# rpng/open_vins

Hardware: NVIDIA H100
Metric: msckf_updates_per_sec (higher is better)
Workload: dtype f64

## Files before the change

open_vins_b200/csrc/chol_tiles.cuh:

```cuda
#pragma once
#include "chol.cuh"
#ifdef CQ_PROBE
#include <cstdio>
#endif

#define CT_XP 12

__device__ __forceinline__ void ct_dmma(double &d0, double &d1, double a, double b) {
  asm volatile("mma.sync.aligned.m8n8k4.row.col.f64.f64.f64.f64 {%0,%1}, {%2}, {%3}, {%0,%1};" : "+d"(d0), "+d"(d1) : "d"(a), "d"(b));
}
__device__ __forceinline__ void ct_dmma2(double &d0, double &d1, double &e0, double &e1, double a0, double a1, double b) {
  asm volatile("mma.sync.aligned.m16n8k4.row.col.f64.f64.f64.f64 {%0,%1,%2,%3}, {%4,%5}, {%6}, {%0,%1,%2,%3};"
               : "+d"(d0), "+d"(d1), "+d"(e0), "+d"(e1)
               : "d"(a0), "d"(a1), "d"(b));
}
__device__ __forceinline__ void ct_dmma2k8(double &d0, double &d1, double &e0, double &e1, double a00, double a01, double a10, double a11, double b0, double b1) {
  asm volatile("mma.sync.aligned.m16n8k8.row.col.f64.f64.f64.f64 {%0,%1,%2,%3}, {%4,%5,%6,%7}, {%8,%9}, {%0,%1,%2,%3};"
               : "+d"(d0), "+d"(d1), "+d"(e0), "+d"(e1)
               : "d"(a00), "d"(a10), "d"(a01), "d"(a11), "d"(b0), "d"(b1));
}
__device__ __forceinline__ int ct_tri(int b) { return (b * (b + 1)) >> 1; }
__device__ __forceinline__ void ct_bar_group(int id, int nthreads) { asm volatile("bar.sync %0, %1;" ::"r"(id), "r"(nthreads) : "memory"); }
__device__ __forceinline__ size_t ct_idx(int i, int j) { return (size_t)(ct_tri(i >> 3) + (j >> 3)) * 64 + (i & 7) * 8 + (j & 7); }

struct CtView {
  double *T, *Xp0, *Xp1, *invd, *Linv0, *Linv1, *dummyT, *dummyX;
  int *flag;
};
__host__ __device__ inline size_t ct_view_doubles(int NRB) {
  return (size_t)((NRB * (NRB + 1)) / 2) * 64 + 2 * (size_t)NRB * 8 * CT_XP + (size_t)NRB * 8 + 128 + 64 + 2 * CT_XP;
}
__device__ __forceinline__ CtView ct_view_carve(double *base, int NRB, int *flag_word) {
  CtView v;
  v.T = base;
  v.Xp0 = v.T + (size_t)((NRB * (NRB + 1)) / 2) * 64;
  v.Xp1 = v.Xp0 + (size_t)NRB * 8 * CT_XP;
  v.invd = v.Xp1 + (size_t)NRB * 8 * CT_XP;
  v.Linv0 = v.invd + (size_t)NRB * 8;
  v.Linv1 = v.Linv0 + 64;
  v.dummyT = v.Linv1 + 64;
  v.dummyX = v.dummyT + 64;
  v.flag = flag_word;
  return v;
}

__device__ __forceinline__ void ct_diag8_frag(double &d0, double &d1, int nbk, double *invd, bool strict, double floor_d, int *flag) {
  const unsigned full = 0xffffffffu;
  const int lane = threadIdx.x & 31, g = lane >> 2, q = lane & 3;
  bool bad = false;
  double myinv = 0.0;
  const double inv_floor = (floor_d > 0.0) ? fast_rsqrt(floor_d) : 0.0;
  double pj = __shfl_sync(full, d0, 0);
#pragma unroll
  for (int j = 0; j < 8; j++) {
    const int jq = j >> 1;
    const double cur = (j & 1) ? d1 : d0;
    const double ag = __shfl_sync(full, cur, 4 * g + jq);
    const double ac0 = __shfl_sync(full, cur, 8 * q + jq);
    const double ac1 = __shfl_sync(full, cur, 8 * q + 4 + jq);
    double an = 0.0, dn = 0.0;
    if (j < 7) {
      an = __shfl_sync(full, cur, 4 * (j + 1) + jq);
      dn = __shfl_sync(full, ((j + 1) & 1) ? d1 : d0, 4 * (j + 1) + ((j + 1) >> 1));
    }
    const double y = fast_rsqrt(pj);
    const bool in = j < nbk;
    double d, iv;
    if (strict) {
      const bool pos = pj > 0.0;
      bad = bad || (in && !pos);
      d = pj;
      iv = (in && pos) ? y : 0.0;
    } else {
      const bool above = pj > floor_d;
      d = above ? pj : floor_d;
      iv = in ? (above ? y : inv_floor) : 0.0;
    }
    if (j < 7) {
      const double ln = an * iv;
      pj = fma(-ln, ln, dn);
    }
    if (lane == j)
      myinv = iv;
    if (q == jq) {
      if (j & 1)
        d1 = (g == j) ? d * iv : d1 * iv;
      else
        d0 = (g == j) ? d * iv : d0 * iv;
    }
    const double lg = ag * iv, lc0 = ac0 * iv, lc1 = ac1 * iv;
    if (2 * q > j)
      d0 = fma(-lg, lc0, d0);
    if (2 * q + 1 > j)
      d1 = fma(-lg, lc1, d1);
  }
  if (lane < 8)
    invd[lane] = myinv;
  if (bad && lane == 0)
    *flag = 1;
}

__device__ __forceinline__ void ct_linv8(const double *Lt, const double *invd, double *Linv) {
  const int lane = threadIdx.x & 31, cc = lane & 7;
  double mc[8];
#pragma unroll
  for (int j = 0; j < 8; j++) {
    double s0 = (j == cc) ? 1.0 : 0.0, s1 = 0.0;
#pragma unroll
    for (int t = 0; t < j; t++) {
      if (t & 1)
        s1 = fma(-Lt[j * 8 + t], mc[t], s1);
      else
        s0 = fma(-Lt[j * 8 + t], mc[t], s0);
    }
    mc[j] = (s0 + s1) * invd[j];
  }
  if (lane < 8) {
#pragma unroll
    for (int i = 0; i < 8; i++)
      Linv[i * 8 + cc] = (i >= cc) ? mc[i] : 0.0;
  }
}

__device__ __forceinline__ void ct_panel_pair(const CtView &sm, int i, int i1, bool two, int k, const double *Linv, double *Xb) {
  const int lane = threadIdx.x & 31, g = lane >> 2, q = lane & 3;
  double *t = sm.T + (size_t)(ct_tri(i) + k) * 64;
  double *t1 = sm.T + (size_t)(ct_tri(i1) + k) * 64;
  const double a0 = t[g * 8 + q], a1 = t[g * 8 + q + 4];
  const double a10 = two ? t1[g * 8 + q] : 0.0, a11 = two ? t1[g * 8 + q + 4] : 0.0;
  const double b0 = Linv[g * 8 + q], b1 = Linv[g * 8 + q + 4];
  double2 d = make_double2(0.0, 0.0), e = make_double2(0.0, 0.0);
  ct_dmma2k8(d.x, d.y, e.x, e.y, a0, a1, a10, a11, b0, b1);
  *reinterpret_cast<double2 *>(t + 2 * lane) = d;
  *reinterpret_cast<double2 *>(Xb + (size_t)(8 * i + g) * CT_XP + 2 * q) = d;
  if (two) {
    *reinterpret_cast<double2 *>(t1 + 2 * lane) = e;
    *reinterpret_cast<double2 *>(Xb + (size_t)(8 * i1 + g) * CT_XP + 2 * q) = e;
  }
}

__device__ __forceinline__ void ct_panel_rows(double *T, double *Xp, const double *invd, int i0, int stride, int nrows, int k, int nbk) {
  if (i0 >= nrows)
    return;
  const double *Lk = T + (size_t)(ct_tri(k) + k) * 64;
  double L[8][8], iv[8];
#pragma unroll
  for (int c = 0; c < 8; c++) {
    iv[c] = (c < nbk) ? invd[8 * k + c] : 0.0;
#pragma unroll
    for (int t2 = 0; t2 < 4; t2++) {
      if (2 * t2 < c) {
        const double2 v = *reinterpret_cast<const double2 *>(Lk + c * 8 + 2 * t2);
        L[c][2 * t2] = v.x;
        L[c][2 * t2 + 1] = v.y;
      }
    }
  }
  for (int i = i0; i < nrows; i += stride) {
    double *src = T + (size_t)(ct_tri(i >> 3) + k) * 64 + (i & 7) * 8;
    double v[8], x[8];
    {
      const double2 v01 = *reinterpret_cast<const double2 *>(src), v23 = *reinterpret_cast<const double2 *>(src + 2);
      const double2 v45 = *reinterpret_cast<const double2 *>(src + 4), v67 = *reinterpret_cast<const double2 *>(src + 6);
      v[0] = v01.x, v[1] = v01.y, v[2] = v23.x, v[3] = v23.y, v[4] = v45.x, v[5] = v45.y, v[6] = v67.x, v[7] = v67.y;
    }
#pragma unroll
    for (int c = 0; c < 8; c++) {
      x[c] = (c < nbk) ? v[c] * iv[c] : 0.0;
#pragma unroll
      for (int t = c + 1; t < 8; t++)
        v[t] = fma(-x[c], L[t][c], v[t]);
    }
// ... 186 lines not shown
```

open_vins_b200/csrc/k_ekf.cu:

```cuda
#include "chol.cuh"
#include "ovb_internal.cuh"

#define EK_T 32

__global__ void __launch_bounds__(256) k_ekf_gemm(int mode, const double *__restrict__ P, int ldP, const double *__restrict__ H, int ldH,
                                                  const double *__restrict__ Min, int ldM, const DevUpdateInfo *__restrict__ info, int X, int Y,
                                                  int K, double *__restrict__ Cout, int ldC, double sigma2, const double *__restrict__ Rdiag) {
  OVB_PDL_ENTER();
  __shared__ double As[EK_T][EK_T + 1];
  __shared__ double Bs[EK_T][EK_T + 1];
  const int x0 = blockIdx.x * EK_T, y0 = blockIdx.y * EK_T;
  if (mode == 1 && y0 > x0 + EK_T - 1)
    return;
  const int tid = threadIdx.x, tx = tid & 31, ty = tid >> 5;
  double acc[4] = {0, 0, 0, 0};
  const int *cs = info->col_state;
  for (int j0 = 0; j0 < K; j0 += EK_T) {
    for (int e = tid; e < EK_T * EK_T; e += 256) {
      int jj = e >> 5, q = e & 31;
      int j = j0 + jj;
      double av = 0.0, bv = 0.0;
      if (j < K) {
        if (mode == 0) {
          int a = x0 + q;
          if (a < X)
            av = P[(size_t)cs[j] * ldP + a];
        } else {
          int i = x0 + q;
          if (i < X)
            av = H[(size_t)i * ldH + j];
        }
        if (mode == 0) {
          int i = y0 + q;
          if (i < Y)
            bv = H[(size_t)i * ldH + j];
        } else {
          int k = y0 + q;
          if (k < Y)
            bv = Min[(size_t)cs[j] * ldM + k];
        }
      }
      As[jj][q] = av;
      Bs[jj][q] = bv;
    }
    __syncthreads();
#pragma unroll 8
    for (int jj = 0; jj < EK_T; jj++) {
      double b = Bs[jj][tx];
#pragma unroll
      for (int u = 0; u < 4; u++)
        acc[u] += As[jj][ty + 8 * u] * b;
    }
    __syncthreads();
  }
#pragma unroll
  for (int u = 0; u < 4; u++) {
    int x = x0 + ty + 8 * u, y = y0 + tx;
    if (x < X && y < Y) {
      double v = acc[u];
      if (mode == 1 && x == y)
        v += Rdiag ? Rdiag[x] : sigma2;
      Cout[(size_t)x * ldC + y] = v;
    }
  }
}

__global__ void __launch_bounds__(EKC_THREADS) k_ekf_chol(double *__restrict__ S, int ldS, int r, const double *__restrict__ res, double *__restrict__ w,
                                                   double *__restrict__ invdiag, DevUpdateInfo *__restrict__ info, int use_smem) {
  OVB_PDL_ENTER();
  extern __shared__ __align__(16) double chol_sm[];
  __shared__ int flag;
  __shared__ double invd_sh[16];
  const int tid = threadIdx.x;
  if (tid == 0)
    flag = 0;
  for (int j = tid; j < r; j += EKC_THREADS)
    S[(size_t)r * ldS + j] = res[j];
  __syncthreads();
  double *W = S;
  int ld = ldS;
  const int lane = tid & 31, wid = tid >> 5;
  if (use_smem) {
    ld = r | 1;
    W = chol_sm;
    stage_lower_async<EKC_THREADS>(W, ld, S, (size_t)ldS, r + 1, r);
  }
  chol_lower_block<EKC_THREADS, 4>(W, ld, r, 1, &flag, invd_sh, nullptr, 0.0, invdiag);
  __syncthreads();
  if (use_smem) {
    for (int i = wid; i < r; i += EKC_THREADS / 32) {
      for (int j = lane; j <= i; j += 32)
        S[(size_t)i * ldS + j] = W[i * ld + j];
    }
  }
  for (int j = tid; j < r; j += EKC_THREADS)
    w[j] = W[(size_t)r * ld + j];
  if (tid == 0 && flag)
    info->not_spd = 1;
}

#define TR_ROWS 8
__global__ void __launch_bounds__(32 * TR_ROWS) k_ekf_trsm(const double *__restrict__ M, int ldM, const double *__restrict__ L, int ldL,
                                                           const double *__restrict__ invdiag, int N, int r, double *__restrict__ Yout, int ldY,
                                                           int L_in_smem, const DevUpdateInfo *__restrict__ info) {
  OVB_PDL_ENTER();
  extern __shared__ __align__(16) double tsm[];
  const int lane = threadIdx.x & 31, wid = threadIdx.x >> 5;
  if (info->not_spd)
    return;
  const int ldl = r | 1;
  double *inv_s = tsm + (size_t)TR_ROWS * r;
  double *Ls = inv_s + r;
  for (int e = threadIdx.x; e < r; e += 32 * TR_ROWS)
    inv_s[e] = invdiag[e];
  if (L_in_smem)
    stage_lower_async<32 * TR_ROWS>(Ls, ldl, L, (size_t)ldL, r, r);
  else
    __syncthreads();
  const double *Lp = L_in_smem ? Ls : L;
  const int lp = L_in_smem ? ldl : ldL;
  const int a = blockIdx.x * TR_ROWS + wid;
  if (a >= N)
    return;
  double *y = tsm + (size_t)wid * r;
  for (int t = lane; t < r; t += 32)
    y[t] = M[(size_t)a * ldM + t];
  __syncwarp();
  for (int kb = 0; kb < r; kb += 8) {
    const int nbk = min(8, r - kb);
    double s[8];
#pragma unroll
    for (int c = 0; c < 8; c++)
      s[c] = 0.0;
    for (int t = lane; t < kb; t += 32) {
      const double yt = y[t];
#pragma unroll
      for (int c = 0; c < 8; c++)
        if (c < nbk)
          s[c] += Lp[(size_t)(kb + c) * lp + t] * yt;
    }
#pragma unroll
    for (int o = 16; o > 0; o >>= 1) {
#pragma unroll
      for (int c = 0; c < 8; c++)
        s[c] += __shfl_xor_sync(0xffffffffu, s[c], o);
    }
    double yn[8];
#pragma unroll
    for (int c = 0; c < 8; c++) {
      if (c < nbk) {
        const double *Lr = Lp + (size_t)(kb + c) * lp + kb;
        double v = y[kb + c] - s[c];
#pragma unroll
        for (int t = 0; t < 8; t++)
          if (t + 1 < c)
            v -= Lr[t] * yn[t];
        if (c > 0)
          v -= Lr[c - 1] * yn[c - 1];
        yn[c] = v * inv_s[kb + c];
      }
    }
    __syncwarp();
    if (lane < nbk) {
      double v = yn[0];
#pragma unroll
      for (int c = 1; c < 8; c++)
        v = (lane == c) ? yn[c] : v;
      y[kb + lane] = v;
    }
    __syncwarp();
  }
  for (int t = lane; t < r; t += 32)
    Yout[(size_t)a * ldY + t] = y[t];
}

__global__ void __launch_bounds__(256) k_ekf_downdate(double *__restrict__ P, int ldP, const double *__restrict__ Yin, int ldY, int N, int r,
                                                      const double *__restrict__ w, double *__restrict__ dx, DevUpdateInfo *__restrict__ info) {
  OVB_PDL_ENTER();
  __shared__ double As[EK_T][EK_T + 1];
  __shared__ double Bs[EK_T][EK_T + 1];
  const int a0 = blockIdx.x * EK_T, b0 = blockIdx.y * EK_T;
  if (b0 < a0)
    return;
  const int tid = threadIdx.x, tx = tid & 31, ty = tid >> 5;
  if (info->not_spd) {
    if (a0 == b0 && tid < EK_T && a0 + tid < N)
      dx[a0 + tid] = 0.0;
    return;
  }
  double acc[4] = {0, 0, 0, 0};
  double dxa = 0.0;
  for (int k0 = 0; k0 < r; k0 += EK_T) {
    for (int e = tid; e < EK_T * EK_T; e += 256) {
      int q = e >> 5, kk = e & 31;
      int k = k0 + kk;
      As[kk][q] = (k < r && a0 + q < N) ? Yin[(size_t)(a0 + q) * ldY + k] : 0.0;
      Bs[kk][q] = (k < r && b0 + q < N) ? Yin[(size_t)(b0 + q) * ldY + k] : 0.0;
    }
    __syncthreads();
#pragma unroll 8
    for (int kk = 0; kk < EK_T; kk++) {
      double b = Bs[kk][tx];
#pragma unroll
      for (int u = 0; u < 4; u++)
        acc[u] += As[kk][ty + 8 * u] * b;
    }
    if (a0 == b0 && tid < EK_T) {
      for (int kk = 0; kk < EK_T; kk++)
        if (k0 + kk < r)
          dxa += As[kk][tid] * w[k0 + kk];
    }
    __syncthreads();
  }
#pragma unroll
  for (int u = 0; u < 4; u++) {
    int a = a0 + ty + 8 * u, b = b0 + tx;
    if (a < N && b < N && b >= a) {
      double v = P[(size_t)a * ldP + b] - acc[u];
      P[(size_t)a * ldP + b] = v;
      P[(size_t)b * ldP + a] = v;
      if (a == b && v < 0.0)
        atomicMin(&info->neg_diag_index, a);
      if (!isfinite(v))
        info->nonfinite = 1;
    }
  }
  if (a0 == b0 && tid < EK_T && a0 + tid < N)
    dx[a0 + tid] = dxa;
}

#define EK1_KMAX 160
__device__ __forceinline__ void ek_cpa8(double *dst_smem, const double *src) {
  asm volatile("cp.async.ca.shared.global [%0], [%1], 8;" ::"r"((unsigned)__cvta_generic_to_shared(dst_smem)), "l"(src) : "memory");
}
__global__ void __launch_bounds__(256) k_ekf_gemm1(int mode, const double *__restrict__ P, int ldP, const double *__restrict__ H, int ldH,
                                                   const double *__restrict__ Min, int ldM, const DevUpdateInfo *__restrict__ info, int X, int Y,
                                                   int K, double *__restrict__ Cout, int ldC, double sigma2, const double *__restrict__ Rdiag) {
  OVB_PDL_ENTER();
  extern __shared__ __align__(16) double g1[];
  const int x0 = blockIdx.x * EK_T, y0 = blockIdx.y * EK_T;
  if (mode == 1 && y0 > x0 + EK_T - 1)
    return;
  const int tid = threadIdx.x, tx = tid & 31, ty = tid >> 5;
  const int *cs = info->col_state;
  const int pk = K | 1;
  double *Gs = g1, *Hs = g1 + (size_t)K * 33;
  const double *Gsrc = (mode == 0) ? P : Min;
  const int ldG = (mode == 0) ? ldP : ldM;
  const int g0 = (mode == 0) ? x0 : y0, gmax = (mode == 0) ? X : Y;
  const int h0 = (mode == 0) ? y0 : x0, hmax = (mode == 0) ? Y : X;
  __shared__ int cs_s[EK1_KMAX];
  for (int j = tid; j < K; j += 256)
    cs_s[j] = cs[j];
  __syncthreads();
  for (int e = tid; e < K * 32; e += 256) {
    const int j = e >> 5, a = e & 31;
    if (g0 + a < gmax)
      ek_cpa8(&Gs[j * 33 + a], &Gsrc[(size_t)cs_s[j] * ldG + g0 + a]);
    else
      Gs[j * 33 + a] = 0.0;
  }
  for (int i = ty; i < 32; i += 8)
    for (int j = tx; j < K; j += 32) {
      if (h0 + i < hmax)
        ek_cpa8(&Hs[i * pk + j], &H[(size_t)(h0 + i) * ldH + j]);
      else
        Hs[i * pk + j] = 0.0;
    }
  asm volatile("cp.async.commit_group;" ::: "memory");
  asm volatile("cp.async.wait_group 0;" ::: "memory");
  __syncthreads();
  double acc[4] = {0, 0, 0, 0};
  if (mode == 0) {
    for (int j = 0; j < K; j++) {
      const double gv = Gs[j * 33 + tx];
#pragma unroll
      for (int u = 0; u < 4; u++)
        acc[u] += gv * Hs[(ty + 8 * u) * pk + j];
    }
#pragma unroll
    for (int u = 0; u < 4; u++) {
      const int a = x0 + tx, i = y0 + ty + 8 * u;
      if (a < X && i < Y)
        Cout[(size_t)a * ldC + i] = acc[u];
    }
  } else {
    for (int j = 0; j < K; j++) {
      const double gv = Gs[j * 33 + tx];
#pragma unroll
      for (int u = 0; u < 4; u++)
        acc[u] += Hs[(ty + 8 * u) * pk + j] * gv;
    }
#pragma unroll
    for (int u = 0; u < 4; u++) {
      const int i = x0 + ty + 8 * u, k = y0 + tx;
      if (i < X && k < Y) {
        double v = acc[u];
        if (i == k)
          v += Rdiag ? Rdiag[i] : sigma2;
        Cout[(size_t)i * ldC + k] = v;
      }
    }
  }
}

__global__ void __launch_bounds__(256) k_ekf_downdate1(double *__restrict__ P, int ldP, const double *__restrict__ Yin, int ldY, int N, int r,
                                                       const double *__restrict__ w, double *__restrict__ dx, DevUpdateInfo *__restrict__ info) {
  OVB_PDL_ENTER();
  extern __shared__ __align__(16) double d1[];
  const int a0 = blockIdx.x * EK_T, b0 = blockIdx.y * EK_T;
  if (b0 < a0)
    return;
  const int tid = threadIdx.x, tx = tid & 31, ty = tid >> 5;
  if (info->not_spd) {
    if (a0 == b0 && tid < EK_T && a0 + tid < N)
      dx[a0 + tid] = 0.0;
    return;
  }
  const int pk = r | 1;
  double *As = d1, *Bs = d1 + (size_t)32 * pk, *ws = Bs + (size_t)32 * pk;
  for (int i = ty; i < 32; i += 8)
    for (int k = tx; k < r; k += 32) {
      if (a0 + i < N)
        ek_cpa8(&As[i * pk + k], &Yin[(size_t)(a0 + i) * ldY + k]);
      else
        As[i * pk + k] = 0.0;
      if (b0 + i < N)
        ek_cpa8(&Bs[i * pk + k], &Yin[(size_t)(b0 + i) * ldY + k]);
      else
        Bs[i * pk + k] = 0.0;
    }
  for (int k = tid; k < r; k += 256)
    ek_cpa8(&ws[k], &w[k]);
  asm volatile("cp.async.commit_group;" ::: "memory");
  asm volatile("cp.async.wait_group 0;" ::: "memory");
  __syncthreads();
  double acc[4] = {0, 0, 0, 0};
  for (int k = 0; k < r; k++) {
    const double bv = Bs[tx * pk + k];
#pragma unroll
    for (int u = 0; u < 4; u++)
      acc[u] += As[(ty + 8 * u) * pk + k] * bv;
  }
#pragma unroll
  for (int u = 0; u < 4; u++) {
    const int a = a0 + ty + 8 * u, b = b0 + tx;
    if (a < N && b < N && b >= a) {
      const double v = P[(size_t)a * ldP + b] - acc[u];
      P[(size_t)a * ldP + b] = v;
      P[(size_t)b * ldP + a] = v;
      if (a == b && v < 0.0)
        atomicMin(&info->neg_diag_index, a);
      if (!isfinite(v))
        info->nonfinite = 1;
    }
  }
  if (a0 == b0 && tid < EK_T && a0 + tid < N) {
    double s0 = 0.0, s1 = 0.0;
    int k = 0;
    for (; k + 1 < r; k += 2) {
      s0 += As[tid * pk + k] * ws[k];
      s1 += As[tid * pk + k + 1] * ws[k + 1];
    }
    if (k < r)
      s0 += As[tid * pk + k] * ws[k];
    dx[a0 + tid] = s0 + s1;
  }
}

__global__ void k_ekf_prep(DevUpdateInfo *info, const int *skip, const double *__restrict__ H, int ldH, int r, int n, double *__restrict__ w) {
  OVB_PDL_ENTER();
  const int i = blockIdx.x * blockDim.x + threadIdx.x;
  if (i < r)
    w[i] = H[(size_t)i * ldH + n];
  if (i == 0) {
    info->neg_diag_index = OVB_NO_NEG_DIAG;
    info->not_spd = (skip && *skip) ? 1 : 0;
    info->nonfinite = 0;
  }
}

void launch_ekf_update(ovb_ctx *ctx, const double *H, int ldHm, int r, int n, bool gate_only, double sigma2, const double *Rdiag_dev,
                       const int *skip_dev) {
  const int N = ctx->N;
  const int ld = ctx->ldP;
  double *P = ctx->P[ctx->cur];
  ovb_launch(ctx, k_ekf_prep, dim3(r > 128 ? (r + 127) / 128 : 1), dim3(128), (size_t)(0), ctx->d_info, skip_dev, H, ldHm, r, n, ctx->d_w);
  if (r <= 0 || n <= 0)
    return;
  if (!ctx->attr_done[2]) {
    cudaFuncSetAttribute(k_ekf_chol, cudaFuncAttributeMaxDynamicSharedMemorySize, 200 * 1024);
    cudaFuncSetAttribute(k_ekf_trsm, cudaFuncAttributeMaxDynamicSharedMemorySize, 200 * 1024);
    cudaFuncSetAttribute(k_ekf_gemm1, cudaFuncAttributeMaxDynamicSharedMemorySize, 100 * 1024);
    cudaFuncSetAttribute(k_ekf_downdate1, cudaFuncAttributeMaxDynamicSharedMemorySize, 100 * 1024);
    ctx->attr_done[2] = 1;
  }
  const bool one_shot = ctx->ekf_chol_dmma && n <= EK1_KMAX && r <= EK1_KMAX;
  dim3 g0((N + EK_T - 1) / EK_T, (r + EK_T - 1) / EK_T);
  dim3 g1((r + EK_T - 1) / EK_T, (r + EK_T - 1) / EK_T);
  if (one_shot) {
    const size_t sm01 = sizeof(double) * ((size_t)n * 33 + (size_t)32 * (n | 1));
    ovb_launch(ctx, k_ekf_gemm1, dim3(g0), dim3(256), sm01, 0, P, ld, H, ldHm, nullptr, 0, ctx->d_info, N, r, n, ctx->d_M, ld, 0.0, nullptr);
    ovb_launch(ctx, k_ekf_gemm1, dim3(g1), dim3(256), sm01, 1, P, ld, H, ldHm, ctx->d_M, ld, ctx->d_info, r, r, n, ctx->d_S, ld, sigma2, Rdiag_dev);
  } else {
    ovb_launch(ctx, k_ekf_gemm, dim3(g0), dim3(256), (size_t)(0), 0, P, ld, H, ldHm, nullptr, 0, ctx->d_info, N, r, n, ctx->d_M, ld, 0.0, nullptr);
    ovb_launch(ctx, k_ekf_gemm, dim3(g1), dim3(256), (size_t)(0), 1, P, ld, H, ldHm, ctx->d_M, ld, ctx->d_info, r, r, n, ctx->d_S, ld, sigma2, Rdiag_dev);
  }
  size_t chol_bytes = sizeof(double) * (size_t)(r + 1) * (size_t)(r | 1);
  int use_smem = chol_bytes <= 200 * 1024;
  double *invdiag = ctx->d_w + ctx->cfg.max_state;
  double *Lpk = nullptr;
  unsigned long long epoch = 0;
  const bool dmma_chol = ctx->ekf_chol_dmma && launch_chol_ekf_dmma(ctx, ctx->d_S, ld, r, ctx->d_w, ctx->d_w, invdiag, &Lpk, gate_only ? nullptr : &epoch);
  const bool wide = !dmma_chol && ctx->ekf_chol_dmma && r < ld && launch_chol_solve_wide(ctx, ctx->d_S, ld, r, ctx->d_w, invdiag, ctx->d_M, ld, N, gate_only);
  if (wide) {
    if (gate_only)
      return;
    dim3 g2w((N + EK_T - 1) / EK_T, (N + EK_T - 1) / EK_T);
    ovb_launch(ctx, k_ekf_downdate, dim3(g2w), dim3(256), (size_t)(0), P, ld, (const double *)ctx->d_M, ld, N, r, ctx->d_w, ctx->d_dx, ctx->d_info);
    return;
  }
  if (!dmma_chol)
    ovb_launch(ctx, k_ekf_chol, dim3(1), dim3(EKC_THREADS), (size_t)(use_smem ? chol_bytes : 0), ctx->d_S, ld, r, ctx->d_w, ctx->d_w, invdiag, ctx->d_info, use_smem);
  if (gate_only)
    return;
  const double *Yd = ctx->d_Y;
  if (dmma_chol && Lpk != nullptr && launch_trsm_rows(ctx, ctx->d_M, ld, N, r, Lpk, epoch)) {
    Yd = ctx->d_M;
  } else {
    size_t trsm_small = sizeof(double) * ((size_t)TR_ROWS * r + r);
    size_t trsm_full = trsm_small + sizeof(double) * (size_t)r * (size_t)(r | 1);
    int L_in_smem = trsm_full <= 200 * 1024;
    ovb_launch(ctx, k_ekf_trsm, dim3((N + TR_ROWS - 1) / TR_ROWS), dim3(32 * TR_ROWS), (size_t)(L_in_smem ? trsm_full : trsm_small), ctx->d_M, ld, ctx->d_S, ld, invdiag, N,
               r, ctx->d_Y, ld, L_in_smem, ctx->d_info);
  }
  dim3 g2((N + EK_T - 1) / EK_T, (N + EK_T - 1) / EK_T);
  if (one_shot) {
    const size_t smd = sizeof(double) * ((size_t)64 * (r | 1) + r);
    ovb_launch(ctx, k_ekf_downdate1, dim3(g2), dim3(256), smd, P, ld, Yd, ld, N, r, ctx->d_w, ctx->d_dx, ctx->d_info);
  } else {
    ovb_launch(ctx, k_ekf_downdate, dim3(g2), dim3(256), (size_t)(0), P, ld, Yd, ld, N, r, ctx->d_w, ctx->d_dx, ctx->d_info);
  }
}


__global__ void k_cov_init_augment(double *__restrict__ P, int ld, int N_max, int k, int n, const DevUpdateInfo *__restrict__ info,
                                   const double *__restrict__ Hx, const double *__restrict__ Hinv, double sigma2, const int *__restrict__ skip,
                                   const int *__restrict__ N_dev) {
  extern __shared__ double ism[];
  double *m = ism, *M = ism + (size_t)N_max * k;
  OVB_PDL_ENTER();
  const int tid = threadIdx.x;
  if (skip && *skip)
    return;
  const int N = N_dev ? *N_dev : N_max;
  for (int a = tid; a < N; a += blockDim.x) {
    for (int i = 0; i < k; i++) {
      double acc = 0.0;
      for (int j = 0; j < n; j++)
        acc += P[(size_t)a * ld + info->col_state[j]] * Hx[i * n + j];
      m[a * k + i] = acc;
    }
  }
  __syncthreads();
  if (tid < k * k) {
    const int i = tid / k, i2 = tid % k;
    double acc = 0.0;
    for (int j = 0; j < n; j++)
      acc += Hx[i * n + j] * m[info->col_state[j] * k + i2];
    M[i * k + i2] = acc + (i == i2 ? sigma2 : 0.0);
  }
  __syncthreads();
  if (tid < k * k) {
    const int i = tid / k, i2 = tid % k;
    if (i2 < i)
      M[i * k + i2] = M[i2 * k + i];
  }
  __syncthreads();
  for (int a = tid; a < N; a += blockDim.x) {
    for (int q = 0; q < k; q++) {
      double acc = 0.0;
      for (int i = 0; i < k; i++)
        acc += m[a * k + i] * Hinv[q * k + i];
      P[(size_t)a * ld + N + q] = -acc;
      P[(size_t)(N + q) * ld + a] = -acc;
    }
  }
  if (tid < k * k) {
    const int q = tid / k, q2 = tid % k;
    double acc = 0.0;
    for (int i = 0; i < k; i++)
      for (int i2 = 0; i2 < k; i2++)
        acc += Hinv[q * k + i] * M[i * k + i2] * Hinv[q2 * k + i2];
    if (q <= q2) {
      P[(size_t)(N + q) * ld + N + q2] = acc;
      P[(size_t)(N + q2) * ld + N + q] = acc;
    }
  }
}

bool launch_cov_init_augment(ovb_ctx *ctx, int k, int n, const double *Hx_dev, const double *Hinv_dev, double sigma2, const int *skip_dev,
                             const int *N_dev) {
  const int N = ctx->N;
  size_t smem = sizeof(double) * ((size_t)N * k + (size_t)k * k);
  if (smem > 200 * 1024)
    return false;
  if (!ctx->attr_done[5]) {
    cudaFuncSetAttribute(k_cov_init_augment, cudaFuncAttributeMaxDynamicSharedMemorySize, 200 * 1024);
    ctx->attr_done[5] = 1;
  }
  return ovb_launch(ctx, k_cov_init_augment, dim3(1), dim3(256), smem, ctx->P[ctx->cur], ctx->ldP, N, k, n, ctx->d_info, Hx_dev, Hinv_dev, sigma2,
                    skip_dev, N_dev) == cudaSuccess;
}

__global__ void k_init_prep(const DevFeat *__restrict__ feat, DevInitSys *__restrict__ sys, DevUpdateInfo *__restrict__ info, int k, int n) {
  OVB_PDL_ENTER();
  const int tid = threadIdx.x;
  const bool ok = feat->status == OVB_FEAT_OK;
  if (ok)
    for (int j = tid; j < n; j += blockDim.x)
      info->col_state[j] = sys->col_state[j];
  if (tid != 0)
    return;
  sys->status = feat->status;
  sys->chi2 = feat->chi2;
  int fail = sys->n != n ? 2 : 0;
  const int o = 3 - k;
  double A[9], Inv[9];
  for (int i = 0; i < k; i++)
    for (int j = 0; j < k; j++) {
      A[i * k + j] = sys->HL[(o + i) * 3 + o + j];
      Inv[i * k + j] = (i == j) ? 1.0 : 0.0;
    }
  for (int c0 = 0; c0 < k && !fail; c0++) {
    int piv = c0;
    for (int i = c0 + 1; i < k; i++)
      if (fabs(A[i * k + c0]) > fabs(A[piv * k + c0]))
        piv = i;
    if (!(fabs(A[piv * k + c0]) > 0.0)) {
      fail = 1;
      break;
    }
    if (piv != c0)
      for (int j = 0; j < k; j++) {
        double t = A[c0 * k + j];
        A[c0 * k + j] = A[piv * k + j];
        A[piv * k + j] = t;
        t = Inv[c0 * k + j];
        Inv[c0 * k + j] = Inv[piv * k + j];
        Inv[piv * k + j] = t;
      }
    const double d = A[c0 * k + c0];
    for (int j = 0; j < k; j++) {
      A[c0 * k + j] /= d;
      Inv[c0 * k + j] /= d;
    }
    for (int i = 0; i < k; i++) {
      if (i == c0)
        continue;
      const double f = A[i * k + c0];
      for (int j = 0; j < k; j++) {
        A[i * k + j] -= f * A[c0 * k + j];
        Inv[i * k + j] -= f * Inv[c0 * k + j];
      }
    }
  }
  for (int q = 0; q < 3; q++) {
    double acc = 0.0;
    if (q < k)
      for (int i = 0; i < k; i++)
        acc += Inv[q * k + i] * sys->res[o + i];
    sys->dx_new[q] = acc;
  }
  for (int i = 0; i < k * k; i++)
    sys->Hinv[i] = Inv[i];
  sys->fail = ok ? fail : 0;
  sys->skip = (!ok || fail) ? 1 : 0;
}

void launch_init_prep(ovb_ctx *ctx, int feat, int k, int n) {
  ovb_launch(ctx, k_init_prep, dim3(1), dim3(256), (size_t)0, ctx->d_feat + feat, ctx->d_init, ctx->d_info, k, n);
}

__global__ void k_cov_clone(double *P, int ld, int N, int old_off, int size, const int *neg_diag) {
  OVB_PDL_ENTER();
  int idx = blockIdx.x * blockDim.x + threadIdx.x;
  int N2 = N + size;
  if (idx >= N2 * size || (neg_diag && *neg_diag != OVB_NO_NEG_DIAG))
    return;
  int i = idx / size, j = idx % size;
  double v;
  if (i < N)
    v = P[(size_t)i * ld + old_off + j];
// ... 268 lines not shown
```

Before: 2708.

## Use FP64 DMMA m16n8k16 tiles for EKF gemm and downdate kernels

Replaces the scalar FMA 32x32 tiles in the one-shot EKF gemm and downdate kernels with 16x8 tiles computed by one warp using the m16n8k16 FP64 mma instruction, with K padded to 16. Staging goes through cp.async with padded shared layouts, and PDL wait/launch_dependents placement is adjusted so H staging overlaps the previous kernel. Smaller tiles raise the block count and let only one warp do the math while the other warps just stage data. The risks are the extra padding work, possible bank conflicts, and whether the m16n8k16 f64 shape is supported on this architecture.

```diff
diff --git a/open_vins_b200/csrc/chol_tiles.cuh b/open_vins_b200/csrc/chol_tiles.cuh
--- a/open_vins_b200/csrc/chol_tiles.cuh
+++ b/open_vins_b200/csrc/chol_tiles.cuh
@@ -18,6 +18,13 @@
   asm volatile("mma.sync.aligned.m16n8k8.row.col.f64.f64.f64.f64 {%0,%1,%2,%3}, {%4,%5,%6,%7}, {%8,%9}, {%0,%1,%2,%3};"
                : "+d"(d0), "+d"(d1), "+d"(e0), "+d"(e1)
                : "d"(a00), "d"(a10), "d"(a01), "d"(a11), "d"(b0), "d"(b1));
+}
+__device__ __forceinline__ void ct_dmma2k16(double &d0, double &d1, double &e0, double &e1, const double (&a)[8], const double (&b)[4]) {
+  asm volatile("mma.sync.aligned.m16n8k16.row.col.f64.f64.f64.f64 {%0,%1,%2,%3}, {%4,%5,%6,%7,%8,%9,%10,%11}, {%12,%13,%14,%15}, "
+               "{%0,%1,%2,%3};"
+               : "+d"(d0), "+d"(d1), "+d"(e0), "+d"(e1)
+               : "d"(a[0]), "d"(a[1]), "d"(a[2]), "d"(a[3]), "d"(a[4]), "d"(a[5]), "d"(a[6]), "d"(a[7]), "d"(b[0]), "d"(b[1]), "d"(b[2]),
+                 "d"(b[3]));
 }
 __device__ __forceinline__ int ct_tri(int b) { return (b * (b + 1)) >> 1; }
 __device__ __forceinline__ void ct_bar_group(int id, int nthreads) { asm volatile("bar.sync %0, %1;" ::"r"(id), "r"(nthreads) : "memory"); }
diff --git a/open_vins_b200/csrc/k_ekf.cu b/open_vins_b200/csrc/k_ekf.cu
--- a/open_vins_b200/csrc/k_ekf.cu
+++ b/open_vins_b200/csrc/k_ekf.cu
@@ -1,4 +1,4 @@
-#include "chol.cuh"
+#include "chol_tiles.cuh"
 #include "ovb_internal.cuh"
 
 #define EK_T 32
@@ -230,141 +230,157 @@
 }
 
 #define EK1_KMAX 160
+#define EK1_M 16
+#define EK1_N 8
+#define EK1_T 128
 __device__ __forceinline__ void ek_cpa8(double *dst_smem, const double *src) {
   asm volatile("cp.async.ca.shared.global [%0], [%1], 8;" ::"r"((unsigned)__cvta_generic_to_shared(dst_smem)), "l"(src) : "memory");
 }
-__global__ void __launch_bounds__(256) k_ekf_gemm1(int mode, const double *__restrict__ P, int ldP, const double *__restrict__ H, int ldH,
-                                                   const double *__restrict__ Min, int ldM, const DevUpdateInfo *__restrict__ info, int X, int Y,
-                                                   int K, double *__restrict__ Cout, int ldC, double sigma2, const double *__restrict__ Rdiag) {
-  OVB_PDL_ENTER();
-  extern __shared__ __align__(16) double g1[];
-  const int x0 = blockIdx.x * EK_T, y0 = blockIdx.y * EK_T;
-  if (mode == 1 && y0 > x0 + EK_T - 1)
-    return;
-  const int tid = threadIdx.x, tx = tid & 31, ty = tid >> 5;
-  const int *cs = info->col_state;
-  const int pk = K | 1;
-  double *Gs = g1, *Hs = g1 + (size_t)K * 33;
-  const double *Gsrc = (mode == 0) ? P : Min;
-  const int ldG = (mode == 0) ? ldP : ldM;
-  const int g0 = (mode == 0) ? x0 : y0, gmax = (mode == 0) ? X : Y;
-  const int h0 = (mode == 0) ? y0 : x0, hmax = (mode == 0) ? Y : X;
-  __shared__ int cs_s[EK1_KMAX];
-  for (int j = tid; j < K; j += 256)
-    cs_s[j] = cs[j];
-  __syncthreads();
-  for (int e = tid; e < K * 32; e += 256) {
-    const int j = e >> 5, a = e & 31;
-    if (g0 + a < gmax)
-      ek_cpa8(&Gs[j * 33 + a], &Gsrc[(size_t)cs_s[j] * ldG + g0 + a]);
+__host__ __device__ __forceinline__ int ek1_kpad(int K) { return (K + 15) & ~15; }
+template <int R> __device__ __forceinline__ void ek1_stage_rows(double *dst, int Kp, const double *src, size_t ld, int x0, int xmax, int K) {
+  const int lane = threadIdx.x & 31;
+  for (int x = threadIdx.x >> 5; x < R; x += EK1_T / 32)
+    for (int k = lane; k < Kp; k += 32) {
+      if (x0 + x < xmax && k < K)
+        ek_cpa8(&dst[x * (Kp + 4) + k], &src[(size_t)(x0 + x) * ld + k]);
+      else
+        dst[x * (Kp + 4) + k] = 0.0;
+    }
+}
+template <int R> __device__ __forceinline__ void ek1_stage_cols(double *dst, int Kp, const double *src, size_t ld, const int *cs_s, int x0, int xmax, int K) {
+  const int x = threadIdx.x % R;
+  for (int k = threadIdx.x / R; k < Kp; k += EK1_T / R) {
+    if (x0 + x < xmax && k < K)
+      ek_cpa8(&dst[k * (R + 4) + x], &src[(size_t)cs_s[k] * ld + x0 + x]);
     else
-      Gs[j * 33 + a] = 0.0;
-  }
-  for (int i = ty; i < 32; i += 8)
-    for (int j = tx; j < K; j += 32) {
-      if (h0 + i < hmax)
-        ek_cpa8(&Hs[i * pk + j], &H[(size_t)(h0 + i) * ldH + j]);
-      else
-        Hs[i * pk + j] = 0.0;
-    }
+      dst[k * (R + 4) + x] = 0.0;
+  }
+}
+__device__ __forceinline__ void ek1_stage_wait() {
   asm volatile("cp.async.commit_group;" ::: "memory");
   asm volatile("cp.async.wait_group 0;" ::: "memory");
   __syncthreads();
-  double acc[4] = {0, 0, 0, 0};
-  if (mode == 0) {
-    for (int j = 0; j < K; j++) {
-      const double gv = Gs[j * 33 + tx];
-#pragma unroll
-      for (int u = 0; u < 4; u++)
-        acc[u] += gv * Hs[(ty + 8 * u) * pk + j];
-    }
+}
+template <bool A_KMAJOR, bool B_KMAJOR> __device__ __forceinline__ void ek1_mma_tile(const double *As, const double *Bs, int Kp, double (&c)[4]) {
+  const int lane = threadIdx.x & 31, g = lane >> 2, q = lane & 3;
+  const int asx = A_KMAJOR ? 1 : Kp + 4, ask = A_KMAJOR ? EK1_M + 4 : 1;
+  const int bsx = B_KMAJOR ? 1 : Kp + 4, bsk = B_KMAJOR ? EK1_N + 4 : 1;
+  const double *ap = As + g * asx + q * ask, *bp = Bs + g * bsx + q * bsk;
+  c[0] = c[1] = c[2] = c[3] = 0.0;
+#pragma unroll 2
+  for (int kb = 0; kb < Kp; kb += 16) {
+    double a[8], b[4];
+#pragma unroll
+    for (int i = 0; i < 8; i++)
+      a[i] = ap[8 * (i & 1) * asx + (kb + 4 * (i >> 1)) * ask];
+#pragma unroll
+    for (int j = 0; j < 4; j++)
+      b[j] = bp[(kb + 4 * j) * bsk];
+    ct_dmma2k16(c[0], c[1], c[2], c[3], a, b);
+  }
+}
+
+__global__ void __launch_bounds__(EK1_T) k_ekf_gemm1(int mode, const double *__restrict__ P, int ldP, const double *__restrict__ H, int ldH,
+                                                     const double *__restrict__ Min, int ldM, const DevUpdateInfo *__restrict__ info, int X, int Y,
+                                                     int K, double *__restrict__ Cout, int ldC, double sigma2, const double *__restrict__ Rdiag) {
+  if (mode == 0)
+    asm volatile("griddepcontrol.wait;" ::: "memory");
+  asm volatile("griddepcontrol.launch_dependents;" ::: "memory");
+  extern __shared__ __align__(16) double g1[];
+  __shared__ int cs_s[EK1_KMAX];
+  const int x0 = blockIdx.x * EK1_M, y0 = blockIdx.y * EK1_N;
+  if (mode == 1 && y0 > x0 + EK1_M - 1)
+    return;
+  const int tid = threadIdx.x, lane = tid & 31, g = lane >> 2, q = lane & 3;
+  const int Kp = ek1_kpad(K);
+  double *As = g1, *Bs = g1 + (size_t)Kp * (EK1_M + 4);
+  if (mode == 0)
+    ek1_stage_rows<EK1_N>(Bs, Kp, H, (size_t)ldH, y0, Y, K);
+  else
+    ek1_stage_rows<EK1_M>(As, Kp, H, (size_t)ldH, x0, X, K);
+  const int *cs = info->col_state;
+  for (int j = tid; j < K; j += EK1_T)
+    cs_s[j] = cs[j];
+  if (mode == 1)
+    asm volatile("griddepcontrol.wait;" ::: "memory");
+  __syncthreads();
+  if (mode == 0)
+    ek1_stage_cols<EK1_M>(As, Kp, P, (size_t)ldP, cs_s, x0, X, K);
+  else
+    ek1_stage_cols<EK1_N>(Bs, Kp, Min, (size_t)ldM, cs_s, y0, Y, K);
+  ek1_stage_wait();
+  if (tid >= 32)
+    return;
+  double c[4];
+  if (mode == 0)
+    ek1_mma_tile<true, false>(As, Bs, Kp, c);
+  else
+    ek1_mma_tile<false, true>(As, Bs, Kp, c);
+#pragma unroll
+  for (int u = 0; u < 4; u++) {
+    const int x = x0 + g + 8 * (u >> 1), y = y0 + 2 * q + (u & 1);
+    if (x < X && y < Y) {
+      double v = c[u];
+      if (mode == 1 && x == y)
+        v += Rdiag ? Rdiag[x] : sigma2;
+      Cout[(size_t)x * ldC + y] = v;
+    }
+  }
+}
+
+__global__ void __launch_bounds__(EK1_T, 1) k_ekf_downdate1(double *__restrict__ P, int ldP, const double *__restrict__ Yin, int ldY, int N, int r,
+                                                         const double *__restrict__ w, double *__restrict__ dx, DevUpdateInfo *__restrict__ info) {
+  OVB_PDL_ENTER();
+  extern __shared__ __align__(16) double d1[];
+  const int a0 = blockIdx.x * EK1_M, b0 = blockIdx.y * EK1_N;
+  if (b0 + EK1_N - 1 < a0)
+    return;
+  const int tid = threadIdx.x, lane = tid & 31, wid = tid >> 5, g = lane >> 2, q = lane & 3;
+  const bool dx_tile = b0 == a0;
+  const int Kp = ek1_kpad(r);
+  double *As = d1, *Bs = As + (size_t)EK1_M * (Kp + 4), *ws = Bs + (size_t)EK1_N * (Kp + 4);
+  ek1_stage_rows<EK1_M>(As, Kp, Yin, (size_t)ldY, a0, N, r);
+  ek1_stage_rows<EK1_N>(Bs, Kp, Yin, (size_t)ldY, b0, N, r);
+  if (dx_tile)
+    for (int k = tid; k < r; k += EK1_T)
+      ek_cpa8(&ws[k], &w[k]);
+  double pv[4];
+#pragma unroll
+  for (int u = 0; u < 4; u++) {
+    const int a = a0 + g + 8 * (u >> 1), b = b0 + 2 * q + (u & 1);
+    pv[u] = (wid == 0 && a < N && b < N && b >= a) ? P[(size_t)a * ldP + b] : 0.0;
+  }
+  const int not_spd = info->not_spd;
+  ek1_stage_wait();
+  if (not_spd) {
+    if (dx_tile && tid < EK1_M && a0 + tid < N)
+      dx[a0 + tid] = 0.0;
+    return;
+  }
+  if (wid == 0) {
+    double c[4];
+    ek1_mma_tile<false, false>(As, Bs, Kp, c);
 #pragma unroll
     for (int u = 0; u < 4; u++) {
-      const int a = x0 + tx, i = y0 + ty + 8 * u;
-      if (a < X && i < Y)
-        Cout[(size_t)a * ldC + i] = acc[u];
-    }
-  } else {
-    for (int j = 0; j < K; j++) {
-      const double gv = Gs[j * 33 + tx];
-#pragma unroll
-      for (int u = 0; u < 4; u++)
-        acc[u] += Hs[(ty + 8 * u) * pk + j] * gv;
-    }
-#pragma unroll
-    for (int u = 0; u < 4; u++) {
-      const int i = x0 + ty + 8 * u, k = y0 + tx;
-      if (i < X && k < Y) {
-        double v = acc[u];
-        if (i == k)
-          v += Rdiag ? Rdiag[i] : sigma2;
-        Cout[(size_t)i * ldC + k] = v;
+      const int a = a0 + g + 8 * (u >> 1), b = b0 + 2 * q + (u & 1);
+      if (a < N && b < N && b >= a) {
+        const double v = pv[u] - c[u];
+        P[(size_t)a * ldP + b] = v;
+        P[(size_t)b * ldP + a] = v;
+        if (a == b && v < 0.0)
+          atomicMin(&info->neg_diag_index, a);
+        if (!isfinite(v))
+          info->nonfinite = 1;
       }
     }
-  }
-}
-
-__global__ void __launch_bounds__(256) k_ekf_downdate1(double *__restrict__ P, int ldP, const double *__restrict__ Yin, int ldY, int N, int r,
-                                                       const double *__restrict__ w, double *__restrict__ dx, DevUpdateInfo *__restrict__ info) {
-  OVB_PDL_ENTER();
-  extern __shared__ __align__(16) double d1[];
-  const int a0 = blockIdx.x * EK_T, b0 = blockIdx.y * EK_T;
-  if (b0 < a0)
-    return;
-  const int tid = threadIdx.x, tx = tid & 31, ty = tid >> 5;
-  if (info->not_spd) {
-    if (a0 == b0 && tid < EK_T && a0 + tid < N)
-      dx[a0 + tid] = 0.0;
-    return;
-  }
-  const int pk = r | 1;
-  double *As = d1, *Bs = d1 + (size_t)32 * pk, *ws = Bs + (size_t)32 * pk;
-  for (int i = ty; i < 32; i += 8)
-    for (int k = tx; k < r; k += 32) {
-      if (a0 + i < N)
-        ek_cpa8(&As[i * pk + k], &Yin[(size_t)(a0 + i) * ldY + k]);
-      else
-        As[i * pk + k] = 0.0;
-      if (b0 + i < N)
-        ek_cpa8(&Bs[i * pk + k], &Yin[(size_t)(b0 + i) * ldY + k]);
-      else
-        Bs[i * pk + k] = 0.0;
-    }
-  for (int k = tid; k < r; k += 256)
-    ek_cpa8(&ws[k], &w[k]);
-  asm volatile("cp.async.commit_group;" ::: "memory");
-  asm volatile("cp.async.wait_group 0;" ::: "memory");
-  __syncthreads();
-  double acc[4] = {0, 0, 0, 0};
-  for (int k = 0; k < r; k++) {
-    const double bv = Bs[tx * pk + k];
-#pragma unroll
-    for (int u = 0; u < 4; u++)
-      acc[u] += As[(ty + 8 * u) * pk + k] * bv;
-  }
-#pragma unroll
-  for (int u = 0; u < 4; u++) {
-    const int a = a0 + ty + 8 * u, b = b0 + tx;
-    if (a < N && b < N && b >= a) {
-      const double v = P[(size_t)a * ldP + b] - acc[u];
-      P[(size_t)a * ldP + b] = v;
-      P[(size_t)b * ldP + a] = v;
-      if (a == b && v < 0.0)
-        atomicMin(&info->neg_diag_index, a);
-      if (!isfinite(v))
-        info->nonfinite = 1;
-    }
-  }
-  if (a0 == b0 && tid < EK_T && a0 + tid < N) {
-    double s0 = 0.0, s1 = 0.0;
-    int k = 0;
-    for (; k + 1 < r; k += 2) {
-      s0 += As[tid * pk + k] * ws[k];
-      s1 += As[tid * pk + k + 1] * ws[k + 1];
-    }
-    if (k < r)
-      s0 += As[tid * pk + k] * ws[k];
-    dx[a0 + tid] = s0 + s1;
+  } else if (wid == 1 && dx_tile) {
+    const double *Ar = As + (lane & 15) * (Kp + 4);
+    double s = 0.0;
+    for (int k = lane >> 4; k < r; k += 2)
+      s = fma(Ar[k], ws[k], s);
+    const double s1 = __shfl_down_sync(0xffffffffu, s, 16);
+    if (lane < EK1_M && a0 + lane < N)
+      dx[a0 + lane] = s + s1;
   }
 }
 
@@ -396,13 +412,14 @@
     ctx->attr_done[2] = 1;
   }
   const bool one_shot = ctx->ekf_chol_dmma && n <= EK1_KMAX && r <= EK1_KMAX;
-  dim3 g0((N + EK_T - 1) / EK_T, (r + EK_T - 1) / EK_T);
-  dim3 g1((r + EK_T - 1) / EK_T, (r + EK_T - 1) / EK_T);
   if (one_shot) {
-    const size_t sm01 = sizeof(double) * ((size_t)n * 33 + (size_t)32 * (n | 1));
-    ovb_launch(ctx, k_ekf_gemm1, dim3(g0), dim3(256), sm01, 0, P, ld, H, ldHm, nullptr, 0, ctx->d_info, N, r, n, ctx->d_M, ld, 0.0, nullptr);
-    ovb_launch(ctx, k_ekf_gemm1, dim3(g1), dim3(256), sm01, 1, P, ld, H, ldHm, ctx->d_M, ld, ctx->d_info, r, r, n, ctx->d_S, ld, sigma2, Rdiag_dev);
+    const size_t sm01 = sizeof(double) * (size_t)ek1_kpad(n) * (EK1_M + 4 + EK1_N + 4);
+    const dim3 t0((N + EK1_M - 1) / EK1_M, (r + EK1_N - 1) / EK1_N), t1((r + EK1_M - 1) / EK1_M, (r + EK1_N - 1) / EK1_N);
+    ovb_launch(ctx, k_ekf_gemm1, t0, dim3(EK1_T), sm01, 0, P, ld, H, ldHm, nullptr, 0, ctx->d_info, N, r, n, ctx->d_M, ld, 0.0, nullptr);
+    ovb_launch(ctx, k_ekf_gemm1, t1, dim3(EK1_T), sm01, 1, P, ld, H, ldHm, ctx->d_M, ld, ctx->d_info, r, r, n, ctx->d_S, ld, sigma2, Rdiag_dev);
   } else {
+    dim3 g0((N + EK_T - 1) / EK_T, (r + EK_T - 1) / EK_T);
+    dim3 g1((r + EK_T - 1) / EK_T, (r + EK_T - 1) / EK_T);
     ovb_launch(ctx, k_ekf_gemm, dim3(g0), dim3(256), (size_t)(0), 0, P, ld, H, ldHm, nullptr, 0, ctx->d_info, N, r, n, ctx->d_M, ld, 0.0, nullptr);
     ovb_launch(ctx, k_ekf_gemm, dim3(g1), dim3(256), (size_t)(0), 1, P, ld, H, ldHm, ctx->d_M, ld, ctx->d_info, r, r, n, ctx->d_S, ld, sigma2, Rdiag_dev);
   }
@@ -434,11 +451,12 @@
     ovb_launch(ctx, k_ekf_trsm, dim3((N + TR_ROWS - 1) / TR_ROWS), dim3(32 * TR_ROWS), (size_t)(L_in_smem ? trsm_full : trsm_small), ctx->d_M, ld, ctx->d_S, ld, invdiag, N,
                r, ctx->d_Y, ld, L_in_smem, ctx->d_info);
   }
-  dim3 g2((N + EK_T - 1) / EK_T, (N + EK_T - 1) / EK_T);
   if (one_shot) {
-    const size_t smd = sizeof(double) * ((size_t)64 * (r | 1) + r);
-    ovb_launch(ctx, k_ekf_downdate1, dim3(g2), dim3(256), smd, P, ld, Yd, ld, N, r, ctx->d_w, ctx->d_dx, ctx->d_info);
+    const size_t smd = sizeof(double) * ((size_t)(EK1_M + EK1_N) * (ek1_kpad(r) + 4) + r);
+    const dim3 t2((N + EK1_M - 1) / EK1_M, (N + EK1_N - 1) / EK1_N);
+    ovb_launch(ctx, k_ekf_downdate1, t2, dim3(EK1_T), smd, P, ld, Yd, ld, N, r, ctx->d_w, ctx->d_dx, ctx->d_info);
   } else {
+    dim3 g2((N + EK_T - 1) / EK_T, (N + EK_T - 1) / EK_T);
     ovb_launch(ctx, k_ekf_downdate, dim3(g2), dim3(256), (size_t)(0), P, ld, Yd, ld, N, r, ctx->d_w, ctx->d_dx, ctx->d_info);
   }
 }
```

Measured after the change: 2820, median of 6. 1.04x the previous value.
